# kokutoupan/webgpu-raytracer

Measured on AMD Instinct MI355X. Metric: Mrays/s (primary+secondary) at 1920x1080 SPP=64 depth=8, higher is better.
Workload: dtype f32; 1 GPU; cornell box 1920x1080, 64 spp as 1 spp x 64 compute() frames (frame_count 1..64, issued as batched dispatches of 32 frames), depth 8, one present() per image; scene=cornell, width=1920, height=1080, spp=64, max_depth=8, parallelism=1 GPU, frames_per_dispatch=32, rays_per_image=645120913

## Files before the change

webgpu-raytracer_amd/csrc/k_intersect.hip.h:

```cpp
#ifndef MI355RT_K_INTERSECT_HIP_H
#define MI355RT_K_INTERSECT_HIP_H

namespace rtk {

struct LocalRay {
  rt3 o, d, inv_d, o_inv_d;
};
__device__ __forceinline__ LocalRay make_ray(rt3 o, rt3 d) {
  LocalRay r;
  r.o = o;
  r.d = d;
  r.inv_d = rt_rcp3(d);
  r.o_inv_d = o * r.inv_d;
  return r;
}
__device__ __forceinline__ bool hit_box(float4 lo, float4 hi, const LocalRay& r, float t_min, float t_max) {
  float t1x = lo.x * r.inv_d.x - r.o_inv_d.x, t2x = hi.x * r.inv_d.x - r.o_inv_d.x;
  float t1y = lo.y * r.inv_d.y - r.o_inv_d.y, t2y = hi.y * r.inv_d.y - r.o_inv_d.y;
  float t1z = lo.z * r.inv_d.z - r.o_inv_d.z, t2z = hi.z * r.inv_d.z - r.o_inv_d.z;
  float nx = rt_min(t1x, t2x), ny = rt_min(t1y, t2y), nz = rt_min(t1z, t2z);
  float fx = rt_max(t1x, t2x), fy = rt_max(t1y, t2y), fz = rt_max(t1z, t2z);
  float tm_near = rt_max(t_min, rt_max(nx, rt_max(ny, nz)));
  float tm_far = rt_min(t_max, rt_min(fx, rt_min(fy, fz)));
  return tm_near <= tm_far;
// ... 55 lines not shown
            uint32_t bdata = rt_f2u(bhi.w);
            if (bdata != 0u) {
              uint32_t first = bdata >> 3, count = bdata & 7u;
              for (uint32_t i = 0; i < count; i++) {
                uint32_t tri = first + i;
                if (COUNT) c.tris++;
                float t = hit_tri(S.tri_geom[RT_TRI_STRIDE * tri], S.tri_geom[RT_TRI_STRIDE * tri + 1], S.tri_geom[RT_TRI_STRIDE * tri + 2], rl, t_min,
                                  closest);
                if (t > 0.0f) {
                  closest = t;
                  best = (int32_t)tri;
                }
              }
            } else {
              bnext = bc + 1u;
            }
          }
          bc = bnext;
        }
        if (best >= 0) {
          res.t = closest;
          res.tri = best;
          res.inst = (int32_t)inst;
        }
      } else {
        next = curr + 1u;
      }
    }
    curr = next;
  }
  return res;
}

template <bool COUNT>
__device__ bool trace_any(const DevScene& S, uint32_t blas_base, rt3 o, rt3 d, float t_min, float t_max,
                          LaneCounters& c) {
  if (blas_base == 0u) return false;
  LocalRay rw = make_ray(o, d);
  uint32_t curr = 0u;
  const uint32_t end_node = rt_f2u(S.nodes[0].w);
  while (curr < end_node) {
    float4 lo = S.nodes[2 * curr], hi = S.nodes[2 * curr + 1];
    if (COUNT) c.nodes++;
    uint32_t next = rt_f2u(lo.w);
    if (hit_box(lo, hi, rw, t_min, t_max)) {
      uint32_t data = rt_f2u(hi.w);
      if (data != 0u) {
        uint32_t inst = data >> 3;
        InvRows m = load_inv_rows(S, inst);
        LocalRay rl = make_ray(mul_point(m, o), mul_dir(m, d));
        const uint32_t start = blas_base + rt_f2u(m.tail.x);
        const uint32_t bend = start + rt_f2u(S.nodes[2 * start].w);
        uint32_t bc = start;
        while (bc < bend) {
          float4 blo = S.nodes[2 * bc], bhi = S.nodes[2 * bc + 1];
          if (COUNT) c.nodes++;
          uint32_t bnext = start + rt_f2u(blo.w);
          if (hit_box(blo, bhi, rl, t_min, t_max)) {
            uint32_t bdata = rt_f2u(bhi.w);
            if (bdata != 0u) {
              uint32_t first = bdata >> 3, count = bdata & 7u;
              for (uint32_t i = 0; i < count; i++) {
                uint32_t tri = first + i;
                if (COUNT) c.tris++;
                float t = hit_tri(S.tri_geom[RT_TRI_STRIDE * tri], S.tri_geom[RT_TRI_STRIDE * tri + 1], S.tri_geom[RT_TRI_STRIDE * tri + 2], rl, t_min,
                                  t_max);
// ... 20 lines not shown
```

webgpu-raytracer_amd/csrc/k_prepare_primary.hip.h:

```cpp
#ifndef MI355RT_K_PREPARE_PRIMARY_HIP_H
#define MI355RT_K_PREPARE_PRIMARY_HIP_H

namespace rtk {

__global__ void k_prepare_tris(const float4* __restrict__ topo, const float4* __restrict__ pos,
                               float4* __restrict__ tri_geom, uint32_t n_tris, uint32_t n_verts) {
  uint32_t i = blockIdx.x * blockDim.x + threadIdx.x;
  if (i >= n_tris) return;
  float4 idx = topo[5 * i];
  uint32_t i0 = rt_f2u(idx.x), i1 = rt_f2u(idx.y), i2 = rt_f2u(idx.z);
  if (i0 >= n_verts) i0 = n_verts - 1;
  if (i1 >= n_verts) i1 = n_verts - 1;
  if (i2 >= n_verts) i2 = n_verts - 1;
  rt3 v0 = xyz(pos[i0]), v1 = xyz(pos[i1]), v2 = xyz(pos[i2]);
  rt3 e1 = v1 - v0, e2 = v2 - v0;
  tri_geom[RT_TRI_STRIDE * i + 0] = make_float4(v0.x, v0.y, v0.z, 0.0f);
  tri_geom[RT_TRI_STRIDE * i + 1] = make_float4(e1.x, e1.y, e1.z, 0.0f);
  tri_geom[RT_TRI_STRIDE * i + 2] = make_float4(e2.x, e2.y, e2.z, 0.0f);
}
__global__ void k_prepare_tri_shade(const float4* __restrict__ topo, const float4* __restrict__ nrm,
                                    const float2* __restrict__ uv, float4* __restrict__ tri_shade, uint32_t n_tris,
                                    uint32_t n_verts) {
  uint32_t i = blockIdx.x * blockDim.x + threadIdx.x;
  if (i >= n_tris) return;
// ... 40 lines not shown
  if (inst >= n_inst) inst = n_inst - 1;
  const InvRows m = load_inv_rows(S, inst);
  const rt3 e1 = xyz(S.tri_geom[RT_TRI_STRIDE * i + 1]), e2 = xyz(S.tri_geom[RT_TRI_STRIDE * i + 2]);
  const rt3 geom_n = rt_normalize(normal_to_world(m, rt_normalize(rt_cross(e1, e2))));
  const WorldTri w = world_triangle(S, i, inst);
  const rt3 edge1 = w.v1 - w.v0;
  const rt3 edge2 = w.v2 - w.v0;
  const rt3 cr = rt_cross(edge1, edge2);
  const float area = rt_length(cr) * 0.5f;
  const rt3 normal = rt_normalize(cr);
  tri_world[2 * i + 0] = make_float4(geom_n.x, geom_n.y, geom_n.z, area);
  tri_world[2 * i + 1] = make_float4(normal.x, normal.y, normal.z, 0.0f);
  const float4* ts = S.tri_shade + 8 * (size_t)i;
  float4* dst = tri_shade_w + 8 * (size_t)i;
  for (int k = 0; k < 4; k++) dst[k] = ts[k];
  for (int k = 4; k < 7; k++) {
    const float4 q = ts[k];
    const rt3 wn = rt_normalize(normal_to_world(m, xyz(q)));
    dst[k] = make_float4(wn.x, wn.y, wn.z, q.w);
  }
  dst[7] = ts[7];
}
__global__ void k_prepare_instances(const float4* __restrict__ inst, float4* __restrict__ inst_trav, uint32_t n) {
  uint32_t i = blockIdx.x * blockDim.x + threadIdx.x;
  if (i >= n) return;
  float4 c0 = inst[9 * i + 4], c1 = inst[9 * i + 5], c2 = inst[9 * i + 6], c3 = inst[9 * i + 7];
  float4 meta = inst[9 * i + 8];
  inst_trav[4 * i + 0] = make_float4(c0.x, c1.x, c2.x, c3.x);
  inst_trav[4 * i + 1] = make_float4(c0.y, c1.y, c2.y, c3.y);
  inst_trav[4 * i + 2] = make_float4(c0.z, c1.z, c2.z, c3.z);
  inst_trav[4 * i + 3] = make_float4(meta.x, c0.w, c1.w, c2.w);
}

template <bool DETAIL, bool LDS>
__global__ __launch_bounds__(LDS ? 256 : 64) void k_primary_visibility(DevScene Sg, DevFrame F, rt_scene_uniforms U,
                                                                       const DevFrameSlot* __restrict__ slots, uint32_t n_tiles,
                                                                       uint32_t n_nodes_total, uint32_t n_tris_total,
                                                                       uint32_t n_inst_total, uint32_t n_verts_total,
                                                                       const float4* __restrict__ tri_shade_w) {
  extern __shared__ float4 s_primary[];
  DevScene S = Sg;
  if (LDS) {
    float4* dst = s_primary;
    auto stage = [&](const void* src, size_t slots_n) {
      const float4* g = reinterpret_cast<const float4*>(src);
      float4* base = dst;
      for (uint32_t i = threadIdx.x; i < slots_n; i += 256) base[i] = g[i];
      dst += slots_n;
      return base;
    };
    S.nodes = stage(Sg.nodes, (size_t)2 * n_nodes_total);
    S.tri_geom = stage(Sg.tri_geom, (size_t)RT_TRI_STRIDE * n_tris_total);
    S.inst_trav = stage(Sg.inst_trav, (size_t)4 * n_inst_total);
    S.tri_shade = stage(tri_shade_w ? tri_shade_w : Sg.tri_shade, (size_t)8 * n_tris_total);
    __syncthreads();
  }
  const uint32_t tile_id = LDS ? blockIdx.x * 4u + (threadIdx.x >> 6) : blockIdx.x;
  const uint32_t lane_id = threadIdx.x & 63u;
  if (slots) {
    const DevFrameSlot sl = slots[blockIdx.y];
    U.frame_count = sl.frame_count;
    U.jitter[0] = sl.jitter_x;
    U.jitter[1] = sl.jitter_y;
    F.albedo = sl.albedo;
    F.normal_id = sl.normal_id;
    F.depth = sl.depth;
  }
  uint32_t x, y;
  bool live;
  if (F.own_period) {
    const uint32_t tiles_x = (U.width + 7u) / 8u;
    uint32_t trow = tile_id / tiles_x;
    trow = (trow / F.own_run) * F.own_period + F.own_first + (trow % F.own_run);
    x = (tile_id % tiles_x) * 8u + (lane_id & 7u);
    y = trow * 8u + (lane_id >> 3);
    live = x < U.width && y < U.height;
  } else {
    live = tile_pixel(U, tile_id, lane_id, x, y) && owns_row(F, y);
  }
  live = live && tile_id < n_tiles;
  LaneCounters c = {0, 0, 0, 0, 0, 0};
  if (live) {
    const uint32_t p_idx = y * U.width + x;
    rt3 eye = rt3_make(U.camera.origin[0], U.camera.origin[1], U.camera.origin[2]);
    rt3 ll = rt3_make(U.camera.lower_left[0], U.camera.lower_left[1], U.camera.lower_left[2]);
    rt3 hor = rt3_make(U.camera.horizontal[0], U.camera.horizontal[1], U.camera.horizontal[2]);
    rt3 ver = rt3_make(U.camera.vertical[0], U.camera.vertical[1], U.camera.vertical[2]);
    rt3 center = ll + hor * 0.5f + ver * 0.5f;
    float focal_length = rt_length(center - eye);
    const float z_near = 0.001f, z_far = 10000.0f;
    float u = ((float)x + 0.5f + U.jitter[0] * (float)U.width) / (float)U.width;
    float v = 1.0f - ((float)y + 0.5f + U.jitter[1] * (float)U.height) / (float)U.height;
    rt3 d = ll + u * hor + v * ver - eye;
    c.primary = 1;
    Hit hit = trace_closest<DETAIL>(S, U.blas_base_idx, eye, d, z_near / focal_length, z_far / focal_length, c);
    if (hit.inst < 0) {
      F.albedo[p_idx] = 0u;
      F.normal_id[p_idx] = make_float4(0.0f, 0.0f, 0.0f, 0.0f);
      F.depth[p_idx] = 1.0f;
    } else {
      InvRows m = load_inv_rows(S, (uint32_t)hit.inst);
      Bary b = barycentrics(S, (uint32_t)hit.tri, mul_point(m, eye), mul_dir(m, d));
      const float4* ts = S.tri_shade + 8 * (size_t)hit.tri;
      const float4 d0 = ts[0], d2 = ts[2], q4 = ts[4], q5 = ts[5], q6 = ts[6], q7 = ts[7];
      rt3 wn0 = xyz(q4), wn1 = xyz(q5), wn2 = xyz(q6);
      if (!LDS || !tri_shade_w) {
        wn0 = rt_normalize(normal_to_world(m, wn0));
        wn1 = rt_normalize(normal_to_world(m, wn1));
        wn2 = rt_normalize(normal_to_world(m, wn2));
      }
      rt3 n = rt_normalize(wn0 * b.w + wn1 * b.u + wn2 * b.v);
      rt2 pn = pack_normal(n);
      rt3 albedo = xyz(d0);
      if (d2.x > -0.5f) {
        rt2 tuv = rt2_make(q4.w, q5.w) * b.w + rt2_make(q6.w, q7.x) * b.u + rt2_make(q7.y, q7.z) * b.v;
        albedo = albedo * sample_tex(S, tuv, rt_f2i32_sat(d2.x));
      }
      F.albedo[p_idx] = rt_unorm8(albedo.x) | (rt_unorm8(albedo.y) << 8) | (rt_unorm8(albedo.z) << 16) | (255u << 24);
      F.normal_id[p_idx] = make_float4(pn.x, pn.y, rt_u2f((uint32_t)hit.tri), rt_u2f((uint32_t)hit.inst));
      float z_view = hit.t * focal_length;
      float z_clip = z_view * (z_far / (z_far - z_near)) - (z_far * z_near) / (z_far - z_near);
      F.depth[p_idx] = z_clip / z_view;
    }
  }
  flush_counters<DETAIL>(c, F.counters, tile_id + blockIdx.y * 977u);
}

}
#endif
```

webgpu-raytracer_amd/csrc/launch_plan.h:

```cpp
#ifndef MI355RT_LAUNCH_PLAN_H
#define MI355RT_LAUNCH_PLAN_H

#include <algorithm>
#include <cstddef>
#include <cstdint>

#include "lds_sizes.h"

namespace launch_plan {

using rtk::LdsPlan;
using rtk::PairPlan;

struct SceneSize {
  uint32_t n_nodes, n_pairs, n_tris, n_inst, n_verts, n_lights, n_tlas;
};
struct PlanKnobs {
  size_t lds_per_cu = 160 * 1024;
  bool no_lds_staging = false;
  long treelet_cap = -1;
  int walk = 2;
  int wf_block = 0;
  int wf_blocks_per_cu = 0;
  int wf_rayreg = -1;
  bool plain_materials = true;
  bool leaf_sweep = true;
  uint32_t leaf_sweep_cap = 16;
  bool leaf_sweep_guard = false;
};
struct SceneFacts {
  bool known = false, plain = false;
};
struct WalkFacts {
  bool known = false, sweepable = false;
  uint32_t n_leaves = 0;
};

struct StagedBytes {
  size_t recs, tris, inst;
  size_t all() const { return recs + tris + inst; }
};
inline StagedBytes node_walk_bytes(const SceneSize& s) {
  return {(size_t)32 * s.n_nodes, (size_t)16 * RT_TRI_STRIDE * s.n_tris, (size_t)64 * s.n_inst + (((size_t)s.n_inst + 3) / 4) * 16};
}
inline StagedBytes pair_walk_bytes(const SceneSize& s) {
  return {(size_t)64 * s.n_pairs, (size_t)16 * RT_TRI_STRIDE * s.n_tris, (size_t)96 * s.n_inst};
}

inline size_t scene_lds_slots(const SceneSize& s) {
  return node_walk_bytes(s).all() / 16 + (size_t)8 * s.n_tris + (size_t)5 * s.n_tris + (size_t)s.n_verts + ((size_t)s.n_verts + 1) / 2 +
         (size_t)9 * s.n_inst + ((size_t)s.n_lights + 1) / 2 + (size_t)4 * s.n_lights;
}
inline size_t one_leaf_lds_slots(const SceneSize& s) {
  return node_walk_bytes(s).all() / 16 + (size_t)8 * s.n_tris + (size_t)2 * s.n_tris + ((size_t)s.n_lights + 1) / 2 + (size_t)4 * s.n_lights;
}
inline size_t primary_lds_slots(const SceneSize& s) {
  const StagedBytes b = node_walk_bytes(s);
  return (b.recs + b.tris) / 16 + (size_t)4 * s.n_inst + (size_t)8 * s.n_tris;
}

inline size_t scene_lds_bytes(const SceneSize& s) { return scene_lds_slots(s) * 16; }
// ... 53 lines not shown
  LdsPlan plan;
  bool plain = false;
  bool sweep = false;
};
inline PersistentShape persistent_plan(const SceneSize& s, const PlanKnobs& k) {
  const size_t queue_bytes = (size_t)4 * RT_WORK_BYTES_PER_WAVE;
  PersistentShape P = {scene_fits_lds(s, k), false, false, 4u, 0, full_lds_plan(s), false};
  if (P.lds)
    P.dyn = queue_bytes + scene_lds_bytes(s);
  else
    P.plan = plan_lds(s, k, k.lds_per_cu / 6, queue_bytes, &P.dyn);
  return P;
}
inline PersistentShape persistent_shape(const SceneSize& s, const PlanKnobs& k, uint32_t n_frames, bool detailed,
                                        const SceneFacts& facts = SceneFacts(), const WalkFacts& walk = WalkFacts()) {
  PersistentShape P = persistent_plan(s, k);
  P.one_inst = one_leaf_lds(s, k);
  if (!P.one_inst) return P;
  const size_t staged_lds = one_leaf_lds_slots(s) * 16;
  const size_t wide_blocks = (size_t)8 * (RT_WORK_BYTES_PER_WAVE + RT_PT_COL_BYTES_PER_WAVE);
  P.wide = !detailed && n_frames > 1 && wide_blocks + scene_lds_bytes(s) <= k.lds_per_cu / 3;
  P.waves = P.wide ? 8u : 4u;
  P.dyn = (P.wide ? wide_blocks : (size_t)4 * RT_WORK_BYTES_PER_WAVE) + staged_lds;
  P.plain = P.wide && facts.known && facts.plain && k.plain_materials;
  P.sweep = P.wide && walk.known && walk.sweepable && walk.n_leaves >= 1 && walk.n_leaves <= k.leaf_sweep_cap && k.leaf_sweep;
  return P;
}

struct PrimaryShape {
  bool lds;
  int block;
  uint32_t tiles_per_workgroup;
  size_t dyn;
};
inline PrimaryShape primary_shape(const SceneSize& s, const PlanKnobs& k) {
  const size_t plds = primary_lds_slots(s) * 16;
  if (plds <= 32 * 1024 && !k.no_lds_staging) return {true, 256, 4u, plds};
  return {false, 64, 1u, 0};
}

struct TraceShape {
  bool pairs, trace_lds, rayreg;
  int block, blocks_per_cu;
  size_t dyn;
  PairPlan plan;
  LdsPlan nplan;
  int rq_form;
};
inline TraceShape trace_shape(const SceneSize& s, const PlanKnobs& k, int wf_block) {
  TraceShape T;
  T.pairs = walks_pairs(s, k);
  const size_t wave_bytes = T.pairs ? RT_PW_BYTES_PER_WAVE : RT_WORK_BYTES_PER_WAVE;
  const size_t lds_records = (T.pairs ? pair_walk_bytes(s) : node_walk_bytes(s)).all();
  T.trace_lds = scene_fits_lds(s, k) && lds_records + (size_t)4 * wave_bytes <= 64 * 1024;
  T.block = 256;
  T.blocks_per_cu = 0;
  if (!T.trace_lds) {
    T.block = wf_block ? wf_block : 256;
    T.blocks_per_cu = k.wf_blocks_per_cu ? k.wf_blocks_per_cu
                      : T.pairs ? std::max(1, std::min((int)(k.lds_per_cu / ((size_t)(T.block / 64) * wave_bytes)), (RT_WF_WAVES * 256) / T.block))
                                : (T.block == 1024 ? 1 : (T.block == 512 ? 2 : 6));
  }
  const size_t queue_bytes = (size_t)(T.block / 64) * wave_bytes;
  T.dyn = queue_bytes + lds_records;
  T.plan = {};
  T.plan.stage_pairs = T.plan.stage_inst = T.plan.stage_tri = 1;
  T.nplan = full_lds_plan(s);
  if (!T.trace_lds) {
    const size_t budget = k.lds_per_cu / (size_t)T.blocks_per_cu;
    if (T.pairs)
      T.plan = plan_pairs(s, k, budget, queue_bytes, &T.dyn);
// ... 13 lines not shown
```

webgpu-raytracer_amd/csrc/lds_sizes.h:

```cpp
#ifndef MI355RT_LDS_SIZES_H
#define MI355RT_LDS_SIZES_H

#include <stdint.h>

#ifndef RT_TRI_STRIDE
#define RT_TRI_STRIDE 3
#endif

#define RT_WORK_BYTES_PER_WAVE (64 * 32 + 64 * 7 * 4 + 64 * 8)

#ifndef RT_PW_STACK_K
#define RT_PW_STACK_K 7
#endif
#define RT_PW_STACK_BYTES_PER_WAVE (RT_PW_STACK_K * 64 * 8)
#define RT_PW_BYTES_PER_WAVE (RT_WORK_BYTES_PER_WAVE + RT_PW_STACK_BYTES_PER_WAVE)

#define RT_PT_COL_BYTES_PER_WAVE (64 * 12)

#ifndef RT_WF_WAVES
#define RT_WF_WAVES 5
#endif

namespace rtk {

struct LdsPlan {
  uint32_t k_nodes, stage_inst, stage_tri, pad;
};

struct TlasRoot {
  float lo[3];
  uint32_t word;
  float hi[3];
  uint32_t pad;
};

struct PairPlan {
  uint32_t stage_pairs, stage_inst, stage_tri, pad;
  TlasRoot troot;
};

enum { RT_RQ_NODE_LDS = 0, RT_RQ_NODE_MIXED = 1, RT_RQ_NODE_RAYREG = 2, RT_RQ_PAIR_LDS = 3, RT_RQ_PAIR_GLOBAL = 4 };

}

#endif
```

webgpu-raytracer_amd/csrc/rt_api.hip:

```cpp

#include <hip/hip_runtime.h>

#include <dlfcn.h>
#include <execinfo.h>

#include <algorithm>
#include <cmath>
#include <cstdio>
#include <cstdlib>
#include <cstring>
#include <deque>
#include <exception>
#include <mutex>
#include <string>
#include <vector>

#include "../../include/mi355rt.h"
#include "kernels.hip.h"
#include "launch_plan.h"
#include "scene_facts.h"
#include "device_owned.h"
#include "bvh_build.hip.h"
#include "world_update.hip.h"
#include "k_ieee_check.hip.h"
// ... 984 lines not shown
  if (hipSetDevice(device_ordinal) != hipSuccess) {
    g_create_error = "hipSetDevice failed";
    return nullptr;
  }
  rt_ctx* c = new rt_ctx();
  c->device = device_ordinal;
  if (hipStreamCreateWithFlags(&c->own_stream, hipStreamNonBlocking) != hipSuccess) {
    g_create_error = "hipStreamCreate failed";
    delete c;
    return nullptr;
  }
  c->stream = c->own_stream;
  if (hipStreamCreateWithFlags(&c->side_stream, hipStreamNonBlocking) != hipSuccess ||
      hipEventCreateWithFlags(&c->side_fork, hipEventDisableTiming) != hipSuccess ||
      hipEventCreateWithFlags(&c->side_join, hipEventDisableTiming) != hipSuccess) {
    g_create_error = "hipStreamCreate / hipEventCreate (side stream) failed";
    delete c;
    return nullptr;
  }
  if (const char* e = getenv("MI355RT_WF_OVERLAP")) c->wf_overlap = atoi(e) != 0;
  if (const char* e = getenv("MI355RT_NO_LDS_STAGING")) c->knobs.no_lds_staging = atoi(e) != 0;
  if (const char* e = getenv("MI355RT_PLAIN_MATERIALS")) c->knobs.plain_materials = atoi(e) != 0;
  if (const char* e = getenv("MI355RT_LEAF_SWEEP")) c->knobs.leaf_sweep = atoi(e) != 0;
  if (const char* e = getenv("MI355RT_LEAF_SWEEP_GUARD")) c->knobs.leaf_sweep_guard = atoi(e) != 0;
  if (const char* e = getenv("MI355RT_SHADE_BLOCKS_PER_CU")) c->shade_per_cu = std::max(1, std::min(4096, atoi(e)));
  if (const char* e = getenv("MI355RT_WF_BLOCK")) {
    const int b = atoi(e);
    if (b == 256 || b == 512 || b == 1024) c->knobs.wf_block = b;
  }
  if (const char* e = getenv("MI355RT_TREELET_MAX")) c->knobs.treelet_cap = atol(e);
  if (const char* e = getenv("MI355RT_TREELET_ORDER")) c->treelet_order = e[0] == 'w' ? 0 : (e[0] == 'i' ? 1 : 2);
  if (const char* e = getenv("MI355RT_WALK")) c->knobs.walk = (e[0] == 'n' || e[0] == '0') ? 0 : ((e[0] == 'a' || e[0] == '2') ? 2 : 1);
  if (const char* e = getenv("MI355RT_WF_RAYREG")) c->knobs.wf_rayreg = atoi(e) != 0 ? 1 : 0;
  if (const char* e = getenv("MI355RT_WF_BLOCKS_PER_CU")) {
    const int b = atoi(e);
    if (b >= 1 && b <= 8) c->knobs.wf_blocks_per_cu = b;
  }
  if (hipMalloc(&c->counters.ptr, 2 * RT_COUNTER_SHARDS * 6 * sizeof(uint64_t)) != hipSuccess) {
    g_create_error = "hipMalloc(counters) failed";
    delete c;
    return nullptr;
  }
  c->counters.capacity = c->counters.size = 2 * RT_COUNTER_SHARDS * 6 * sizeof(uint64_t);
  {
    hipDeviceProp_t prop;
    if (hipGetDeviceProperties(&prop, device_ordinal) == hipSuccess && prop.multiProcessorCount > 0)
      c->num_cus = prop.multiProcessorCount;
    (void)hipMalloc(&c->ticket.ptr, 256);
    c->ticket.capacity = c->ticket.size = 256;
  }
  (void)hipMemsetAsync(c->counters.ptr, 0, c->counters.size, c->stream);
  (void)hipMalloc(&c->lights.ptr, 16);
  c->lights.capacity = 16;
  (void)hipMemsetAsync(c->lights.ptr, 0, 16, c->stream);
  (void)hipStreamSynchronize(c->stream);
  return c;
}

void rt_destroy(rt_ctx* c) {
  if (!c) return;
  (void)hipSetDevice(c->device);
  (void)hipStreamSynchronize(c->stream);
  dist_release(c);
  delete c;
}

const char* rt_last_error(const rt_ctx* c) { return c ? c->error.c_str() : g_create_error.c_str(); }

int rt_set_pipeline(rt_ctx* c, uint32_t max_depth, uint32_t spp) {
  if (!c) return RT_ERR_INVALID;
  c->epoch++;
  if (spp == 0) return fail(c, RT_ERR_INVALID, "SPP must be >= 1");
  c->max_depth = max_depth;
  c->spp = spp;
  c->pipeline_built = true;
  return RT_OK;
}

int rt_resize(rt_ctx* c, uint32_t width, uint32_t height) {
  if (!c) return RT_ERR_INVALID;
// ... 850 lines not shown
  return r ? RT_REALLOCATED : RT_OK;
}

int rt_set_scene(rt_ctx* c, const float camera[24], uint32_t frame_count, uint32_t light_count) {
  if (!c || !camera) return RT_ERR_INVALID;
  c->epoch++;
  c->light_count = light_count;
  step_jitter(c, frame_count, frame_count);
  std::memcpy(&c->uniforms.camera, camera, 96);
  std::memcpy(&c->uniforms.prev_camera, c->prev_camera, 96);
  write_mixed(c, frame_count);
  std::memcpy(c->prev_camera, camera, 96);
  return RT_OK;
}

int rt_recreate_bind_group(rt_ctx* c) { return c ? RT_OK : RT_ERR_INVALID; }

#define RT_WF_TRACE_FNS(K, B)                                                                                          \
  {{{(const void*)K<false, false, false, B>, (const void*)K<false, false, true, B>},                                 \
    {(const void*)K<false, true, false, B>, (const void*)K<false, true, true, B>}},                                  \
   {{(const void*)K<true, false, false, B>, (const void*)K<true, false, true, B>},                                   \
    {(const void*)K<true, true, false, B>, (const void*)K<true, true, true, B>}}}
static const void* const wf_node_fns[3][2][2][2] = {RT_WF_TRACE_FNS(rtk::k_wf_trace, 256), RT_WF_TRACE_FNS(rtk::k_wf_trace, 512),
                                                    RT_WF_TRACE_FNS(rtk::k_wf_trace, 1024)};
static const void* const wf_pair_fns[3][2][2][2] = {RT_WF_TRACE_FNS(rtk::k_wf_trace_pairs, 256),
                                                    RT_WF_TRACE_FNS(rtk::k_wf_trace_pairs, 512),
                                                    RT_WF_TRACE_FNS(rtk::k_wf_trace_pairs, 1024)};
#undef RT_WF_TRACE_FNS
static const void* const wf_node_rayreg_fns[2][2] = {
    {(const void*)rtk::k_wf_trace<false, false, false, 256, true>, (const void*)rtk::k_wf_trace<false, true, false, 256, true>},
    {(const void*)rtk::k_wf_trace<true, false, false, 256, true>, (const void*)rtk::k_wf_trace<true, true, false, 256, true>}};
static const void* const wf_shade_fns[2][2] = {{(const void*)rtk::k_wf_shade<false, false>, (const void*)rtk::k_wf_shade<false, true>},
                                               {(const void*)rtk::k_wf_shade<true, false>, (const void*)rtk::k_wf_shade<true, true>}};
static const void* const primary_fns[2][2] = {
    {(const void*)rtk::k_primary_visibility<false, false>, (const void*)rtk::k_primary_visibility<false, true>},
    {(const void*)rtk::k_primary_visibility<true, false>, (const void*)rtk::k_primary_visibility<true, true>}};
static int launch_wavefront(rt_ctx* c, const DevScene& S, const DevFrame& F, const DevFrameSlot* dslots, uint32_t n) {
  const size_t npx = (size_t)c->width * c->height;
  const size_t items = npx * n;
  if (items >= (1ull << 31)) return fail(c, RT_ERR_INVALID, "batch too large for the wavefront queues");
  int r;
  const uint32_t shade_blocks = (uint32_t)std::min<size_t>((items + 255) / 256, (size_t)c->num_cus * (size_t)c->shade_per_cu);
  const size_t qcap = items + (size_t)shade_blocks * 4 * 256 + 1024 * 1024;
  r = ensure_buffer(c, c->wf_queues, qcap * 132, false);
  if (r < 0) return r;
  r = ensure_buffer(c, c->wf_state, 2 * qcap * sizeof(WfPath), false);
  if (r < 0) return r;
  const uint32_t depths = c->max_depth ? c->max_depth : 1u;
  r = ensure_buffer(c, c->wf_counters, (size_t)(depths + 2) * 32, false);
  if (r < 0) return r;
  HIP_TRY(c, hipMemsetAsync(c->wf_counters.ptr, 0, (size_t)(depths + 2) * 32, c->stream));
  WfState W;
  W.p[0] = (WfPath*)c->wf_state.ptr;
  W.p[1] = W.p[0] + qcap;
  WfQueues Q;
  char* qb = (char*)c->wf_queues.ptr;
  Q.shadow_rays = (float4*)qb;
  Q.ext_rays[0] = (float4*)(qb + qcap * 32);
  Q.ext_rays[1] = (float4*)(qb + qcap * 64);
  Q.ext_hit = (float4*)(qb + qcap * 96);
  Q.active[0] = (uint32_t*)(qb + qcap * 112);
  Q.active[1] = (uint32_t*)(qb + qcap * 116);
  Q.shadow_ids = (uint32_t*)(qb + qcap * 120);
  Q.ext_ids = (uint32_t*)(qb + qcap * 124);
  Q.occluded = (uint32_t*)(qb + qcap * 128);
  Q.counters = (uint32_t*)c->wf_counters.ptr;
  const bool detail = c->detailed_counters;
  lp::TraceShape shape = lp::trace_shape(scene_size(c), c->knobs, c->knobs.wf_block);
  shape.plan.troot = c->troot;
// ... 2122 lines not shown

  DevScene S = dev_scene(c);
  DevFrame F;
  F.accum = accum_ptr(c);
  F.frame_col = (n > 1 || wavefront) ? (float4*)c->frame_col.ptr : nullptr;
  F.albedo = (uint32_t*)c->render_target.ptr;
  F.normal_id = (float4*)c->g_normal.ptr;
  F.depth = (float*)c->g_depth.ptr;
  F.counters = (uint64_t*)c->counters.ptr;
  F.max_depth = c->max_depth;
  F.spp = c->spp;
  F.stripe_rows = c->stripe_rows;
  F.stripe_rank = c->stripe_rank;
  F.stripe_count = c->stripe_count;
  F.own_run = F.own_period = F.own_first = F.own_tile_rows = 0;
  if (c->stripe_count > 1 && c->stripe_rows && c->stripe_rows % 8 == 0) {
    const uint32_t tile_rows = (c->height + 7) / 8;
    F.own_run = c->stripe_rows / 8;
    F.own_period = F.own_run * c->stripe_count;
    F.own_first = F.own_run * c->stripe_rank;
    uint32_t owned = 0;
    for (uint32_t ty = 0; ty < tile_rows; ty++)
      if ((ty / F.own_run) % c->stripe_count == c->stripe_rank) owned++;
    F.own_tile_rows = owned;
  }
  DevFrame Fp = F;
  F.counters = (uint64_t*)c->counters.ptr + (size_t)RT_COUNTER_SHARDS * 6;
  const uint32_t tiles = ((c->width + 7) / 8) * ((c->height + 7) / 8);
  const uint32_t own_tiles = F.own_period ? ((c->width + 7) / 8) * F.own_tile_rows : tiles;

  EventPair* ev = next_events(c, RT_TIMER_PRIMARY);
  if (ev) HIP_TRY(c, hipEventRecord(ev->a, c->stream));
  if (own_tiles) {
    const lp::PrimaryShape shape = lp::primary_shape(size, c->knobs);
    uint32_t nn = c->n_nodes, nt = c->n_tris, ni = c->n_instances, nv = c->n_verts, n_ptiles = own_tiles;
    const float4* tsw = (lp::one_leaf_lds(size, c->knobs) && !c->world_rec_dirty) ? (const float4*)c->tri_shade_w.ptr : nullptr;
    void* args[] = {&S, &Fp, &c->uniforms, &dslots, &n_ptiles, &nn, &nt, &ni, &nv, &tsw};
    const uint32_t per_wg = shape.tiles_per_workgroup;
    HIP_TRY(c, hipLaunchKernel(primary_fns[c->detailed_counters][shape.lds], dim3((own_tiles + per_wg - 1) / per_wg, n),
                               dim3(shape.block), args, shape.dyn, c->stream));
  }
  if (ev) HIP_TRY(c, hipEventRecord(ev->b, c->stream));
  c->gbuf_gen++;
  c->fm.gbuf_scene_gen = c->fm.scene_gen;
  c->albedo_plane_valid = true;
  c->fd.keep_valid = false;
  if (c->fd.wanted && n_commit < n) {
    if ((r = ensure_buffer(c, c->fd.albedo_keep, npx * 4, false)) < 0) return r;
    HIP_TRY(c, hipMemcpyAsync(c->fd.albedo_keep.ptr, c->render_target.ptr, npx * 4, hipMemcpyDeviceToDevice, c->stream));
    c->fd.keep_valid = true;
  }

  c->pt_form = RT_PT_FORM_NONE;
  if (wavefront) {
    r = launch_wavefront(c, S, F, dslots, n);
    if (r < 0) return r;
  } else if (c->variant == 0) {
    r = launch_megakernel(c, S, F, dslots, tiles);
    if (r < 0) return r;
  } else {
    HIP_TRY(c, hipMemsetAsync(c->ticket.ptr, 0, 4, c->stream));
    lp::PersistentShape shape = lp::persistent_shape(size, c->knobs, n, c->detailed_counters, c->facts, c->walk);
    if (shape.one_inst && c->world_rec_dirty) return fail(c, RT_ERR_INTERNAL, "one-leaf form without its world records");
    if (shape.sweep && (c->walk_dirty || !c->leaf_recs.ptr)) return fail(c, RT_ERR_INTERNAL, "sweep form without its leaf records");
    if (shape.sweep && (c->walk_nodes < c->walk.n_leaves || c->walk_nodes > scene_facts::kMaxNodeRecords))
      return fail(c, RT_ERR_INTERNAL, "sweep form without its node records");
    const void* fn = shape.sweep      ? pt_sweep_fns[shape.plain]
                     : shape.plain    ? pt_plain_fn
                     : shape.wide     ? pt_wide_fn
                     : shape.one_inst ? pt_one_leaf_fns[c->detailed_counters]
                                      : pt_fns[c->detailed_counters][shape.lds];
    int per_cu;
// ... 604 lines not shown
```

Before: 29750 Mrays/s.

## Add multi-round tiles-per-wave primary visibility kernel with one-leaf TLAS shortcut

Adds a primary-visibility kernel form in which each wave handles several tiles across rounds. This amortises the LDS staging of scene data and the per-wave setup (camera terms, TLAS leaf and instance matrix) over more work, with the uniform values hoisted into scalar registers via readfirstlane. For one-leaf scenes the TLAS walk is replaced by a single box test, and the triangle test now returns barycentrics so the separate barycentric recomputation is dropped. The round count is picked so the grid still has enough resident rounds per CU. Fewer workgroups may hurt load balance, and the new kernel adds register pressure.

```diff
diff --git a/webgpu-raytracer_amd/csrc/k_intersect.hip.h b/webgpu-raytracer_amd/csrc/k_intersect.hip.h
--- a/webgpu-raytracer_amd/csrc/k_intersect.hip.h
+++ b/webgpu-raytracer_amd/csrc/k_intersect.hip.h
@@ -111,6 +111,107 @@
   return res;
 }
 
+__device__ __forceinline__ float hit_tri_uv(float4 g0, float4 g1, float4 g2, const LocalRay& r, float t_min, float t_max,
+                                            float& u_out, float& v_out) {
+  rt3 v0 = xyz(g0), e1 = xyz(g1), e2 = xyz(g2);
+  rt3 h = rt_cross(r.d, e2);
+  float a = rt_dot(e1, h);
+  if (rt_abs(a) < 1e-6f) return -1.0f;
+  float f = rt_rcp(a);
+  rt3 s = r.o - v0;
+  float u = f * rt_dot(s, h);
+  if (u < 0.0f || u > 1.0f) return -1.0f;
+  rt3 q = rt_cross(s, e1);
+  float v = f * rt_dot(r.d, q);
+  if (v < 0.0f || u + v > 1.0f) return -1.0f;
+  float t = f * rt_dot(e2, q);
+  u_out = u;
+  v_out = v;
+  return (t > t_min && t < t_max) ? t : -1.0f;
+}
+
+struct HitUV {
+  Hit hit;
+  float u, v;
+};
+
+template <bool COUNT>
+__device__ __forceinline__ void walk_blas_uv(const DevScene& S, uint32_t blas_base, const InvRows& m, uint32_t inst, rt3 o, rt3 d,
+                                             float t_min, LaneCounters& c, HitUV& res) {
+  LocalRay rl = make_ray(mul_point(m, o), mul_dir(m, d));
+  const uint32_t start = blas_base + rt_f2u(m.tail.x);
+  const uint32_t bend = start + rt_f2u(S.nodes[2 * start].w);
+  uint32_t bc = start;
+  while (bc < bend) {
+    float4 blo = S.nodes[2 * bc], bhi = S.nodes[2 * bc + 1];
+    if (COUNT) c.nodes++;
+    uint32_t bnext = start + rt_f2u(blo.w);
+    if (hit_box(blo, bhi, rl, t_min, res.hit.t)) {
+      uint32_t bdata = rt_f2u(bhi.w);
+      if (bdata != 0u) {
+        uint32_t first = bdata >> 3, count = bdata & 7u;
+        for (uint32_t i = 0; i < count; i++) {
+          uint32_t tri = first + i;
+          if (COUNT) c.tris++;
+          float tu = 0.0f, tv = 0.0f;
+          float t = hit_tri_uv(S.tri_geom[RT_TRI_STRIDE * tri], S.tri_geom[RT_TRI_STRIDE * tri + 1], S.tri_geom[RT_TRI_STRIDE * tri + 2], rl, t_min,
+                               res.hit.t, tu, tv);
+          if (t > 0.0f) {
+            res.hit.t = t;
+            res.hit.tri = (int32_t)tri;
+            res.hit.inst = (int32_t)inst;
+            res.u = tu;
+            res.v = tv;
+          }
+        }
+      } else {
+        bnext = bc + 1u;
+      }
+    }
+    bc = bnext;
+  }
+}
+
+struct TlasLeaf {
+  float4 lo, hi;
+  InvRows m;
+};
+
+template <bool COUNT, bool ONE_LEAF>
+__device__ __forceinline__ HitUV trace_closest_uv(const DevScene& S, uint32_t blas_base, rt3 o, rt3 d, float t_min, float t_max,
+                                                  LaneCounters& c, const TlasLeaf& L) {
+  HitUV res;
+  res.hit.t = t_max;
+  res.hit.tri = -1;
+  res.hit.inst = -1;
+  res.u = res.v = 0.0f;
+  if (blas_base == 0u) return res;
+  LocalRay rw = make_ray(o, d);
+  if (ONE_LEAF) {
+    if (COUNT) c.nodes++;
+    if (hit_box(L.lo, L.hi, rw, t_min, res.hit.t)) walk_blas_uv<COUNT>(S, blas_base, L.m, rt_f2u(L.hi.w) >> 3, o, d, t_min, c, res);
+    return res;
+  }
+  uint32_t curr = 0u;
+  const uint32_t end_node = rt_f2u(S.nodes[0].w);
+  while (curr < end_node) {
+    float4 lo = S.nodes[2 * curr], hi = S.nodes[2 * curr + 1];
+    if (COUNT) c.nodes++;
+    uint32_t next = rt_f2u(lo.w);
+    if (hit_box(lo, hi, rw, t_min, res.hit.t)) {
+      uint32_t data = rt_f2u(hi.w);
+      if (data != 0u) {
+        uint32_t inst = data >> 3;
+        walk_blas_uv<COUNT>(S, blas_base, load_inv_rows(S, inst), inst, o, d, t_min, c, res);
+      } else {
+        next = curr + 1u;
+      }
+    }
+    curr = next;
+  }
+  return res;
+}
+
 template <bool COUNT>
 __device__ bool trace_any(const DevScene& S, uint32_t blas_base, rt3 o, rt3 d, float t_min, float t_max,
                           LaneCounters& c) {
diff --git a/webgpu-raytracer_amd/csrc/k_prepare_primary.hip.h b/webgpu-raytracer_amd/csrc/k_prepare_primary.hip.h
--- a/webgpu-raytracer_amd/csrc/k_prepare_primary.hip.h
+++ b/webgpu-raytracer_amd/csrc/k_prepare_primary.hip.h
@@ -96,12 +96,17 @@
   inst_trav[4 * i + 3] = make_float4(meta.x, c0.w, c1.w, c2.w);
 }
 
-template <bool DETAIL, bool LDS>
-__global__ __launch_bounds__(LDS ? 256 : 64) void k_primary_visibility(DevScene Sg, DevFrame F, rt_scene_uniforms U,
-                                                                       const DevFrameSlot* __restrict__ slots, uint32_t n_tiles,
-                                                                       uint32_t n_nodes_total, uint32_t n_tris_total,
-                                                                       uint32_t n_inst_total, uint32_t n_verts_total,
-                                                                       const float4* __restrict__ tri_shade_w) {
+__device__ __forceinline__ float wave_uniform(float x, uint32_t zero = 0u) {
+  return rt_u2f((uint32_t)__builtin_amdgcn_readfirstlane((int)(rt_f2u(x) | zero)));
+}
+__device__ __forceinline__ float4 wave_uniform(float4 q) {
+  return make_float4(wave_uniform(q.x), wave_uniform(q.y), wave_uniform(q.z), wave_uniform(q.w));
+}
+template <bool DETAIL, bool LDS, bool TILES>
+__device__ __forceinline__ void primary_visibility(DevScene Sg, DevFrame F, rt_scene_uniforms U, const DevFrameSlot* __restrict__ slots,
+                                                   uint32_t n_tiles, uint32_t n_nodes_total, uint32_t n_tris_total,
+                                                   uint32_t n_inst_total, const float4* __restrict__ tri_shade_w, uint32_t rounds) {
+  static_assert(LDS || !TILES, "the form of many tiles per wave is an LDS form");
   extern __shared__ float4 s_primary[];
   DevScene S = Sg;
   if (LDS) {
@@ -119,8 +124,10 @@
     S.tri_shade = stage(tri_shade_w ? tri_shade_w : Sg.tri_shade, (size_t)8 * n_tris_total);
     __syncthreads();
   }
-  const uint32_t tile_id = LDS ? blockIdx.x * 4u + (threadIdx.x >> 6) : blockIdx.x;
+  const uint32_t wave = TILES ? (uint32_t)__builtin_amdgcn_readfirstlane((int)(threadIdx.x >> 6)) : threadIdx.x >> 6;
   const uint32_t lane_id = threadIdx.x & 63u;
+  const uint32_t n_rounds = TILES ? rounds : 1u;
+  const uint32_t first_tile = LDS ? primary_tile(blockIdx.x, n_rounds, 0u, wave) : blockIdx.x;
   if (slots) {
     const DevFrameSlot sl = slots[blockIdx.y];
     U.frame_count = sl.frame_count;
@@ -130,54 +137,85 @@
     F.normal_id = sl.normal_id;
     F.depth = sl.depth;
   }
-  uint32_t x, y;
-  bool live;
-  if (F.own_period) {
-    const uint32_t tiles_x = (U.width + 7u) / 8u;
-    uint32_t trow = tile_id / tiles_x;
-    trow = (trow / F.own_run) * F.own_period + F.own_first + (trow % F.own_run);
-    x = (tile_id % tiles_x) * 8u + (lane_id & 7u);
-    y = trow * 8u + (lane_id >> 3);
-    live = x < U.width && y < U.height;
-  } else {
-    live = tile_pixel(U, tile_id, lane_id, x, y) && owns_row(F, y);
-  }
-  live = live && tile_id < n_tiles;
+  const rt3 eye = rt3_make(U.camera.origin[0], U.camera.origin[1], U.camera.origin[2]);
+  const rt3 ll = rt3_make(U.camera.lower_left[0], U.camera.lower_left[1], U.camera.lower_left[2]);
+  const rt3 hor = rt3_make(U.camera.horizontal[0], U.camera.horizontal[1], U.camera.horizontal[2]);
+  const rt3 ver = rt3_make(U.camera.vertical[0], U.camera.vertical[1], U.camera.vertical[2]);
+  const rt3 center = ll + hor * 0.5f + ver * 0.5f;
+  float focal_length = rt_length(center - eye);
+  const float z_near = 0.001f, z_far = 10000.0f;
+  float t_near = z_near / focal_length, t_far = z_far / focal_length;
+  float width_f = (float)U.width, height_f = (float)U.height;
+  float jitter_x = U.jitter[0] * width_f, jitter_y = U.jitter[1] * height_f;
+  TlasLeaf leaf = {};
+  if (TILES) {
+    const uint32_t zero = (threadIdx.x >> 6) ^ wave;
+    focal_length = wave_uniform(focal_length, zero);
+    t_near = wave_uniform(t_near, zero);
+    t_far = wave_uniform(t_far, zero);
+    width_f = wave_uniform(width_f, zero);
+    height_f = wave_uniform(height_f, zero);
+    jitter_x = wave_uniform(jitter_x, zero);
+    jitter_y = wave_uniform(jitter_y, zero);
+    if (U.blas_base_idx != 0u) {
+      leaf.lo = wave_uniform(S.nodes[0]);
+      leaf.hi = wave_uniform(S.nodes[1]);
+      const InvRows m = load_inv_rows(S, rt_f2u(leaf.hi.w) >> 3);
+      leaf.m.r0 = wave_uniform(m.r0);
+      leaf.m.r1 = wave_uniform(m.r1);
+      leaf.m.r2 = wave_uniform(m.r2);
+      leaf.m.tail = wave_uniform(m.tail);
+    }
+  }
+  uint32_t n_live = 0;
   LaneCounters c = {0, 0, 0, 0, 0, 0};
-  if (live) {
+  for (uint32_t r = 0; r < n_rounds; r++) {
+    const uint32_t tile_id = first_tile + 4u * r;
+    if (TILES && tile_id >= n_tiles) break;
+    uint32_t x, y;
+    bool live;
+    if (!TILES && F.own_period) {
+      const uint32_t tiles_x = (U.width + 7u) / 8u;
+      uint32_t trow = tile_id / tiles_x;
+      trow = (trow / F.own_run) * F.own_period + F.own_first + (trow % F.own_run);
+      x = (tile_id % tiles_x) * 8u + (lane_id & 7u);
+      y = trow * 8u + (lane_id >> 3);
+      live = x < U.width && y < U.height;
+    } else {
+      live = tile_pixel(U, tile_id, lane_id, x, y) && (TILES || owns_row(F, y));
+    }
+    live = live && tile_id < n_tiles;
+    if (TILES)
+      n_live += (uint32_t)__builtin_popcountll(__builtin_amdgcn_ballot_w64(live));
+    else if (live)
+      c.primary = 1;
+    if (!live) continue;
     const uint32_t p_idx = y * U.width + x;
-    rt3 eye = rt3_make(U.camera.origin[0], U.camera.origin[1], U.camera.origin[2]);
-    rt3 ll = rt3_make(U.camera.lower_left[0], U.camera.lower_left[1], U.camera.lower_left[2]);
-    rt3 hor = rt3_make(U.camera.horizontal[0], U.camera.horizontal[1], U.camera.horizontal[2]);
-    rt3 ver = rt3_make(U.camera.vertical[0], U.camera.vertical[1], U.camera.vertical[2]);
-    rt3 center = ll + hor * 0.5f + ver * 0.5f;
-    float focal_length = rt_length(center - eye);
-    const float z_near = 0.001f, z_far = 10000.0f;
-    float u = ((float)x + 0.5f + U.jitter[0] * (float)U.width) / (float)U.width;
-    float v = 1.0f - ((float)y + 0.5f + U.jitter[1] * (float)U.height) / (float)U.height;
+    float u = ((float)x + 0.5f + jitter_x) / width_f;
+    float v = 1.0f - ((float)y + 0.5f + jitter_y) / height_f;
     rt3 d = ll + u * hor + v * ver - eye;
-    c.primary = 1;
-    Hit hit = trace_closest<DETAIL>(S, U.blas_base_idx, eye, d, z_near / focal_length, z_far / focal_length, c);
+    const HitUV hv = trace_closest_uv<DETAIL, TILES>(S, U.blas_base_idx, eye, d, t_near, t_far, c, leaf);
+    const Hit hit = hv.hit;
     if (hit.inst < 0) {
       F.albedo[p_idx] = 0u;
       F.normal_id[p_idx] = make_float4(0.0f, 0.0f, 0.0f, 0.0f);
       F.depth[p_idx] = 1.0f;
     } else {
-      InvRows m = load_inv_rows(S, (uint32_t)hit.inst);
-      Bary b = barycentrics(S, (uint32_t)hit.tri, mul_point(m, eye), mul_dir(m, d));
+      const float b_u = hv.u, b_v = hv.v, b_w = 1.0f - hv.u - hv.v;
       const float4* ts = S.tri_shade + 8 * (size_t)hit.tri;
       const float4 d0 = ts[0], d2 = ts[2], q4 = ts[4], q5 = ts[5], q6 = ts[6], q7 = ts[7];
       rt3 wn0 = xyz(q4), wn1 = xyz(q5), wn2 = xyz(q6);
       if (!LDS || !tri_shade_w) {
+        const InvRows m = TILES ? leaf.m : load_inv_rows(S, (uint32_t)hit.inst);
         wn0 = rt_normalize(normal_to_world(m, wn0));
         wn1 = rt_normalize(normal_to_world(m, wn1));
         wn2 = rt_normalize(normal_to_world(m, wn2));
       }
-      rt3 n = rt_normalize(wn0 * b.w + wn1 * b.u + wn2 * b.v);
+      rt3 n = rt_normalize(wn0 * b_w + wn1 * b_u + wn2 * b_v);
       rt2 pn = pack_normal(n);
       rt3 albedo = xyz(d0);
       if (d2.x > -0.5f) {
-        rt2 tuv = rt2_make(q4.w, q5.w) * b.w + rt2_make(q6.w, q7.x) * b.u + rt2_make(q7.y, q7.z) * b.v;
+        rt2 tuv = rt2_make(q4.w, q5.w) * b_w + rt2_make(q6.w, q7.x) * b_u + rt2_make(q7.y, q7.z) * b_v;
         albedo = albedo * sample_tex(S, tuv, rt_f2i32_sat(d2.x));
       }
       F.albedo[p_idx] = rt_unorm8(albedo.x) | (rt_unorm8(albedo.y) << 8) | (rt_unorm8(albedo.z) << 16) | (255u << 24);
@@ -187,7 +225,22 @@
       F.depth[p_idx] = z_clip / z_view;
     }
   }
-  flush_counters<DETAIL>(c, F.counters, tile_id + blockIdx.y * 977u);
+  if (TILES) c.primary = lane_id == 0u ? n_live : 0u;
+  flush_counters<DETAIL>(c, F.counters, first_tile + blockIdx.y * 977u);
+}
+template <bool DETAIL, bool LDS>
+__global__ __launch_bounds__(LDS ? 256 : 64) void k_primary_visibility(DevScene Sg, DevFrame F, rt_scene_uniforms U,
+                                                                       const DevFrameSlot* __restrict__ slots, uint32_t n_tiles,
+                                                                       uint32_t n_nodes_total, uint32_t n_tris_total,
+                                                                       uint32_t n_inst_total, uint32_t n_verts_total,
+                                                                       const float4* __restrict__ tri_shade_w, uint32_t rounds) {
+  primary_visibility<DETAIL, LDS, false>(Sg, F, U, slots, n_tiles, n_nodes_total, n_tris_total, n_inst_total, tri_shade_w, rounds);
+}
+template <bool DETAIL>
+__global__ __launch_bounds__(256) __attribute__((amdgpu_num_sgpr(96))) void k_primary_visibility_tiles(
+    DevScene Sg, DevFrame F, rt_scene_uniforms U, const DevFrameSlot* __restrict__ slots, uint32_t n_tiles, uint32_t n_nodes_total,
+    uint32_t n_tris_total, uint32_t n_inst_total, uint32_t n_verts_total, const float4* __restrict__ tri_shade_w, uint32_t rounds) {
+  primary_visibility<DETAIL, true, true>(Sg, F, U, slots, n_tiles, n_nodes_total, n_tris_total, n_inst_total, tri_shade_w, rounds);
 }
 
 }
diff --git a/webgpu-raytracer_amd/csrc/launch_plan.h b/webgpu-raytracer_amd/csrc/launch_plan.h
--- a/webgpu-raytracer_amd/csrc/launch_plan.h
+++ b/webgpu-raytracer_amd/csrc/launch_plan.h
@@ -27,6 +27,8 @@
   bool leaf_sweep = true;
   uint32_t leaf_sweep_cap = 16;
   bool leaf_sweep_guard = false;
+  uint32_t n_cus = 256;
+  uint32_t primary_rounds = 0;
 };
 struct SceneFacts {
   bool known = false, plain = false;
@@ -146,11 +148,25 @@
   int block;
   uint32_t tiles_per_workgroup;
   size_t dyn;
-};
-inline PrimaryShape primary_shape(const SceneSize& s, const PlanKnobs& k) {
+  uint32_t rounds = 1;
+  bool tiles = false;
+};
+constexpr uint32_t PRIMARY_ROUNDS_MAX = 8;
+constexpr uint32_t PRIMARY_MIN_RESIDENT_ROUNDS = 12;
+inline PrimaryShape primary_shape(const SceneSize& s, const PlanKnobs& k, uint64_t tile_frames = 0, bool striped = false) {
   const size_t plds = primary_lds_slots(s) * 16;
-  if (plds <= 32 * 1024 && !k.no_lds_staging) return {true, 256, 4u, plds};
-  return {false, 64, 1u, 0};
+  if (plds > 32 * 1024 || k.no_lds_staging) return {false, 64, 1u, 0, 1u, false};
+  if (!one_leaf_lds(s, k) || striped) return {true, 256, 4u, plds, 1u, false};
+  uint32_t rounds = 1;
+  if (k.primary_rounds)
+    rounds = k.primary_rounds;
+  else
+    while (rounds < PRIMARY_ROUNDS_MAX && tile_frames / ((uint64_t)8 * rounds) >= (uint64_t)PRIMARY_MIN_RESIDENT_ROUNDS * 8 * k.n_cus) rounds *= 2;
+  return {true, 256, 4u, plds, rounds, rounds > 1};
+}
+inline uint32_t primary_grid_x(const PrimaryShape& p, uint32_t own_tiles) {
+  const uint64_t per_wg = (uint64_t)p.tiles_per_workgroup * p.rounds;
+  return (uint32_t)((own_tiles + per_wg - 1) / per_wg);
 }
 
 struct TraceShape {
diff --git a/webgpu-raytracer_amd/csrc/lds_sizes.h b/webgpu-raytracer_amd/csrc/lds_sizes.h
--- a/webgpu-raytracer_amd/csrc/lds_sizes.h
+++ b/webgpu-raytracer_amd/csrc/lds_sizes.h
@@ -39,6 +39,8 @@
   TlasRoot troot;
 };
 
+constexpr uint32_t primary_tile(uint32_t wg, uint32_t rounds, uint32_t r, uint32_t wave) { return (wg * rounds + r) * 4u + wave; }
+
 enum { RT_RQ_NODE_LDS = 0, RT_RQ_NODE_MIXED = 1, RT_RQ_NODE_RAYREG = 2, RT_RQ_PAIR_LDS = 3, RT_RQ_PAIR_GLOBAL = 4 };
 
 }
diff --git a/webgpu-raytracer_amd/csrc/rt_api.hip b/webgpu-raytracer_amd/csrc/rt_api.hip
--- a/webgpu-raytracer_amd/csrc/rt_api.hip
+++ b/webgpu-raytracer_amd/csrc/rt_api.hip
@@ -1040,6 +1040,7 @@
   if (const char* e = getenv("MI355RT_TREELET_ORDER")) c->treelet_order = e[0] == 'w' ? 0 : (e[0] == 'i' ? 1 : 2);
   if (const char* e = getenv("MI355RT_WALK")) c->knobs.walk = (e[0] == 'n' || e[0] == '0') ? 0 : ((e[0] == 'a' || e[0] == '2') ? 2 : 1);
   if (const char* e = getenv("MI355RT_WF_RAYREG")) c->knobs.wf_rayreg = atoi(e) != 0 ? 1 : 0;
+  if (const char* e = getenv("MI355RT_PRIMARY_ROUNDS")) c->knobs.primary_rounds = (uint32_t)std::max(0, std::min(64, atoi(e)));
   if (const char* e = getenv("MI355RT_WF_BLOCKS_PER_CU")) {
     const int b = atoi(e);
     if (b >= 1 && b <= 8) c->knobs.wf_blocks_per_cu = b;
@@ -1054,6 +1055,7 @@
     hipDeviceProp_t prop;
     if (hipGetDeviceProperties(&prop, device_ordinal) == hipSuccess && prop.multiProcessorCount > 0)
       c->num_cus = prop.multiProcessorCount;
+    c->knobs.n_cus = (uint32_t)c->num_cus;
     (void)hipMalloc(&c->ticket.ptr, 256);
     c->ticket.capacity = c->ticket.size = 256;
   }
@@ -1970,9 +1972,11 @@
     {(const void*)rtk::k_wf_trace<true, false, false, 256, true>, (const void*)rtk::k_wf_trace<true, true, false, 256, true>}};
 static const void* const wf_shade_fns[2][2] = {{(const void*)rtk::k_wf_shade<false, false>, (const void*)rtk::k_wf_shade<false, true>},
                                                {(const void*)rtk::k_wf_shade<true, false>, (const void*)rtk::k_wf_shade<true, true>}};
-static const void* const primary_fns[2][2] = {
-    {(const void*)rtk::k_primary_visibility<false, false>, (const void*)rtk::k_primary_visibility<false, true>},
-    {(const void*)rtk::k_primary_visibility<true, false>, (const void*)rtk::k_primary_visibility<true, true>}};
+static const void* const primary_fns[2][3] = {
+    {(const void*)rtk::k_primary_visibility<false, false>, (const void*)rtk::k_primary_visibility<false, true>,
+     (const void*)rtk::k_primary_visibility_tiles<false>},
+    {(const void*)rtk::k_primary_visibility<true, false>, (const void*)rtk::k_primary_visibility<true, true>,
+     (const void*)rtk::k_primary_visibility_tiles<true>}};
 static int launch_wavefront(rt_ctx* c, const DevScene& S, const DevFrame& F, const DevFrameSlot* dslots, uint32_t n) {
   const size_t npx = (size_t)c->width * c->height;
   const size_t items = npx * n;
@@ -4161,12 +4165,16 @@
   EventPair* ev = next_events(c, RT_TIMER_PRIMARY);
   if (ev) HIP_TRY(c, hipEventRecord(ev->a, c->stream));
   if (own_tiles) {
-    const lp::PrimaryShape shape = lp::primary_shape(size, c->knobs);
+    const lp::PrimaryShape shape = lp::primary_shape(size, c->knobs, (uint64_t)own_tiles * n, c->stripe_count > 1 && c->stripe_rows);
     uint32_t nn = c->n_nodes, nt = c->n_tris, ni = c->n_instances, nv = c->n_verts, n_ptiles = own_tiles;
-    const float4* tsw = (lp::one_leaf_lds(size, c->knobs) && !c->world_rec_dirty) ? (const float4*)c->tri_shade_w.ptr : nullptr;
-    void* args[] = {&S, &Fp, &c->uniforms, &dslots, &n_ptiles, &nn, &nt, &ni, &nv, &tsw};
-    const uint32_t per_wg = shape.tiles_per_workgroup;
-    HIP_TRY(c, hipLaunchKernel(primary_fns[c->detailed_counters][shape.lds], dim3((own_tiles + per_wg - 1) / per_wg, n),
+    const bool one_leaf = lp::one_leaf_lds(size, c->knobs);
+    const float4* tsw = (one_leaf && !c->world_rec_dirty) ? (const float4*)c->tri_shade_w.ptr : nullptr;
+    uint32_t rounds = shape.rounds;
+    if (getenv("MI355RT_DEBUG_SHAPE"))
+      fprintf(stderr, "[mi355rt] primary kernel: %s form, %u rounds, grid %u x %u, %zu bytes of LDS\n",
+              shape.lds ? (shape.tiles ? "LDS many-tiles" : "LDS") : "global", rounds, lp::primary_grid_x(shape, own_tiles), (unsigned)n, shape.dyn);
+    void* args[] = {&S, &Fp, &c->uniforms, &dslots, &n_ptiles, &nn, &nt, &ni, &nv, &tsw, &rounds};
+    HIP_TRY(c, hipLaunchKernel(primary_fns[c->detailed_counters][shape.lds ? (shape.tiles ? 2 : 1) : 0], dim3(lp::primary_grid_x(shape, own_tiles), n),
                                dim3(shape.block), args, shape.dyn, c->stream));
   }
   if (ev) HIP_TRY(c, hipEventRecord(ev->b, c->stream));
```

Result: faster. 30150 Mrays/s, median of 6 (+1.4%).
